# crockwell/rel_pose

Hardware: AMD Instinct MI355X
Metric: image-pairs/sec fwd+bwd @384x384, 1/2/4/8 MI355X; R,t err vs ref (higher is better)
Workload: dtype f32; 1 GPU; train.py step (ViTEss fwd + geodesic loss + bwd + grad all-reduce + clip + Adam), synthetic 384x384 pairs; scope=full, pairs_per_gpu=64, global_batch_pairs=64, parallelism=dp1, finite=True, gemm_operand_precision=exact fp32 MFMA, launch=eager

## Files before the change

__graft_entry__.py:

```python
import os
import subprocess
import sys

ROOT = os.path.dirname(os.path.abspath(__file__))
if ROOT not in sys.path:
    sys.path.insert(0, ROOT)


def build():
    import torch
    from rel_pose_amd import _build
    force = os.environ.get("RP_FORCE_BUILD", "" if torch.cuda.is_available() else "1") == "1"
    _build.build(force=force, verbose=True)
    from rel_pose_amd import _lib
    lib = _lib.load()
    assert lib.rp_abi_version() == _lib.ABI_VERSION and lib.rp_target_arch() == b"gfx950"
    assert lib.rp_abi_export_count() == _lib.ABI_EXPORTS == len(_lib.EXPORTS)
    assert _lib.load_readout().rp_readout_abi_version() == _lib.READOUT_ABI_VERSION
    assert _lib.load_eightpoint().rp_eightpoint_abi_version() == _lib.EIGHTPOINT_ABI_VERSION
    assert _lib.load_refine().rp_refine_abi_version() == _lib.REFINE_ABI_VERSION
    assert _lib.load_consensus().rp_consensus_abi_version() == _lib.CONSENSUS_ABI_VERSION
    assert _lib.load_submatch().rp_submatch_abi_version() == _lib.SUBMATCH_ABI_VERSION
    assert _lib.load_fivepoint().rp_fivepoint_abi_version() == _lib.FIVEPOINT_ABI_VERSION
    assert _lib.load_homography().rp_homography_abi_version() == _lib.HOMOGRAPHY_ABI_VERSION
    assert _lib.load_triangulate().rp_triangulate_abi_version() == _lib.TRIANGULATE_ABI_VERSION
    import rel_pose_amd.model
    import oracle.relpose_oracle
    print("build ok:", _lib.lib_path(), _build.READOUT_LIB, _build.EIGHTPOINT_LIB, _build.REFINE_LIB, _build.CONSENSUS_LIB, _build.SUBMATCH_LIB,
          _build.FIVEPOINT_LIB, _build.HOMOGRAPHY_LIB, _build.TRIANGULATE_LIB)


def smoke():
    import types

    import torch

    from oracle import relpose_oracle as O
    from rel_pose_amd import _lib
    from rel_pose_amd.model import ViTEss
    assert torch.cuda.is_available(), "smoke() needs cuda:0"
    _lib.load()
    torch.cuda.set_device(0)
    args = types.SimpleNamespace(noess="", pool_size=60, fc_hidden_size=512, fusion_transformer=True,
                                 transformer_depth=6, cross_features=False, use_single_softmax=False,
                                 no_pos_encoding=False, l1_pos_encoding=False)
    shapes = dict(O.vit_param_shapes())
    shapes.update(O.cnn_param_shapes())
    sd32, sd64 = O.make_state(shapes, torch.float32), O.make_state(shapes, torch.float64)
    model = ViTEss(args)
    model.load_state_dict(sd32)
    model = model.cuda().train()
    tok = O.synthetic_tokens(2)
    Gs = torch.tensor([0, 0, 0, 0, 0, 0, 1.0]).repeat(1, 2, 1)
    intr = torch.tensor([[30.0, 26.0, 12.0, 11.0]]).repeat(1, 2, 1)
    fmap = tok.permute(0, 2, 1).contiguous().view(2, 192, 24, 24).cuda().requires_grad_(True)
    out = model.forward_tokens(fmap, Gs.cuda(), intr.cuda())
    out[:, 1].square().sum().backward()
    t64 = tok.double().requires_grad_(True)
    ref = O.vit_ess_from_tokens(sd64, t64, Gs.double(), intr.double())
    ref[:, 1].square().sum().backward()
    t_err, q_err, ang = O.pose_errors(out.detach().cpu(), ref.detach())
    g_err = O.rel_err(fmap.grad.view(2, 192, 576).permute(0, 2, 1).cpu(), t64.grad)
# ... 10 lines not shown
```

rel_pose_amd/_build.py:

```python
import os
import subprocess
import sys

HERE = os.path.dirname(os.path.abspath(__file__))
CSRC = os.path.join(HERE, "csrc")
LIB = os.path.join(HERE, "librelpose_hip.so")
SOURCES = ["gemm.hip", "gemm_dma.hip", "rowwise.hip", "attention.hip", "attention_bf16.hip", "dw192_bf16.hip", "dw192_f32.hip", "dw192_split3.hip", "dx_lnbwd_bf16.hip", "emm.hip", "emm_bf16.hip", "batchnorm.hip", "se3loss.hip", "geom.hip", "augment.hip", "mlp_fused.hip", "linear_rows.hip", "conv_stem.hip", "conv_stem_bf16.hip", "conv_stem_wgrad_bf16.hip", "conv_stem_wgrad_f32.hip", "conv3x3_bf16.hip", "conv3x3_wgrad_bf16.hip", "conv3x3_wgrad_f32.hip", "conv3x3_f32.hip", "conv3x3_c128_f32.hip"]
READOUT_CSRC = os.path.join(HERE, "csrc_readout")
READOUT_LIB = os.path.join(HERE, "librelpose_readout.so")
READOUT_SOURCES = ["emm_readout.hip"]
EIGHTPOINT_CSRC = os.path.join(HERE, "csrc_eightpoint")
EIGHTPOINT_LIB = os.path.join(HERE, "librelpose_eightpoint.so")
EIGHTPOINT_SOURCES = ["eight_point.hip"]
REFINE_CSRC = os.path.join(HERE, "csrc_refine")
REFINE_LIB = os.path.join(HERE, "librelpose_refine.so")
REFINE_SOURCES = ["refine_pose.hip"]
CONSENSUS_CSRC = os.path.join(HERE, "csrc_consensus")
CONSENSUS_LIB = os.path.join(HERE, "librelpose_consensus.so")
CONSENSUS_SOURCES = ["consensus.hip"]
SUBMATCH_CSRC = os.path.join(HERE, "csrc_submatch")
SUBMATCH_LIB = os.path.join(HERE, "librelpose_submatch.so")
SUBMATCH_SOURCES = ["submatch.hip"]
FIVEPOINT_CSRC = os.path.join(HERE, "csrc_fivepoint")
FIVEPOINT_LIB = os.path.join(HERE, "librelpose_fivepoint.so")
FIVEPOINT_SOURCES = ["five_point.hip"]
HOMOGRAPHY_CSRC = os.path.join(HERE, "csrc_homography")
HOMOGRAPHY_LIB = os.path.join(HERE, "librelpose_homography.so")
HOMOGRAPHY_SOURCES = ["homography.hip"]
TRIANGULATE_CSRC = os.path.join(HERE, "csrc_triangulate")
TRIANGULATE_LIB = os.path.join(HERE, "librelpose_triangulate.so")
TRIANGULATE_SOURCES = ["triangulate.hip"]
ARCH = "gfx950"


def _hipcc():
    for c in (os.environ.get("HIPCC"), "/opt/rocm/bin/hipcc"):
        if c and os.path.exists(c):
            return c
    return "hipcc"


def _stale(lib, csrc, sources, headers):
    if not os.path.exists(lib):
        return True
    t = os.path.getmtime(lib)
    return any(os.path.getmtime(d) > t for d in [os.path.join(csrc, s) for s in sources] + headers)


def needs_build():
    return _stale(LIB, CSRC, SOURCES, _headers())


def readout_needs_build():
    return _stale(READOUT_LIB, READOUT_CSRC, READOUT_SOURCES, _readout_headers())


def eightpoint_needs_build():
    return _stale(EIGHTPOINT_LIB, EIGHTPOINT_CSRC, EIGHTPOINT_SOURCES, _eightpoint_headers())


def refine_needs_build():
    return _stale(REFINE_LIB, REFINE_CSRC, REFINE_SOURCES, _refine_headers())


def consensus_needs_build():
    return _stale(CONSENSUS_LIB, CONSENSUS_CSRC, CONSENSUS_SOURCES, _consensus_headers())


def submatch_needs_build():
    return _stale(SUBMATCH_LIB, SUBMATCH_CSRC, SUBMATCH_SOURCES, _submatch_headers())


def fivepoint_needs_build():
    return _stale(FIVEPOINT_LIB, FIVEPOINT_CSRC, FIVEPOINT_SOURCES, _fivepoint_headers())


def homography_needs_build():
    return _stale(HOMOGRAPHY_LIB, HOMOGRAPHY_CSRC, HOMOGRAPHY_SOURCES, _homography_headers())


def triangulate_needs_build():
    return _stale(TRIANGULATE_LIB, TRIANGULATE_CSRC, TRIANGULATE_SOURCES, _triangulate_headers())


def build(force=False, verbose=True):
    import fcntl
    with open(os.path.join(HERE, ".build.lock"), "w") as lock:
        fcntl.flock(lock, fcntl.LOCK_EX)
        try:
            if force or needs_build():
                _build_locked(verbose, force, LIB, CSRC, SOURCES, _headers())
            if force or readout_needs_build():
                _build_locked(verbose, force, READOUT_LIB, READOUT_CSRC, READOUT_SOURCES, _readout_headers())
            if force or eightpoint_needs_build():
                _build_locked(verbose, force, EIGHTPOINT_LIB, EIGHTPOINT_CSRC, EIGHTPOINT_SOURCES, _eightpoint_headers())
            if force or refine_needs_build():
                _build_locked(verbose, force, REFINE_LIB, REFINE_CSRC, REFINE_SOURCES, _refine_headers())
            if force or consensus_needs_build():
                _build_locked(verbose, force, CONSENSUS_LIB, CONSENSUS_CSRC, CONSENSUS_SOURCES, _consensus_headers())
            if force or submatch_needs_build():
                _build_locked(verbose, force, SUBMATCH_LIB, SUBMATCH_CSRC, SUBMATCH_SOURCES, _submatch_headers())
            if force or fivepoint_needs_build():
                _build_locked(verbose, force, FIVEPOINT_LIB, FIVEPOINT_CSRC, FIVEPOINT_SOURCES, _fivepoint_headers())
            if force or homography_needs_build():
                _build_locked(verbose, force, HOMOGRAPHY_LIB, HOMOGRAPHY_CSRC, HOMOGRAPHY_SOURCES, _homography_headers())
            if force or triangulate_needs_build():
                _build_locked(verbose, force, TRIANGULATE_LIB, TRIANGULATE_CSRC, TRIANGULATE_SOURCES, _triangulate_headers())
            return LIB
        finally:
            fcntl.flock(lock, fcntl.LOCK_UN)


def _headers():
    return [os.path.join(CSRC, h) for h in sorted(os.listdir(CSRC)) if h.endswith(".h")] + \
           [os.path.join(os.path.dirname(HERE), "include", "relpose_hip.h")]


def _readout_headers():
    return _headers() + [os.path.join(os.path.dirname(HERE), "include", "relpose_readout.h")]


def _eightpoint_headers():
    return _headers() + [os.path.join(os.path.dirname(HERE), "include", "relpose_eightpoint.h")]


def _refine_headers():
    return _headers() + [os.path.join(os.path.dirname(HERE), "include", "relpose_refine.h")]


def _consensus_headers():
    return _headers() + [os.path.join(os.path.dirname(HERE), "include", "relpose_consensus.h")]


def _submatch_headers():
    return _headers() + [os.path.join(os.path.dirname(HERE), "include", "relpose_submatch.h")]


def _fivepoint_headers():
    return _headers() + [os.path.join(os.path.dirname(HERE), "include", "relpose_fivepoint.h")]


def _homography_headers():
    return _headers() + [os.path.join(os.path.dirname(HERE), "include", "relpose_homography.h")]


def _triangulate_headers():
    return _headers() + [os.path.join(os.path.dirname(HERE), "include", "relpose_triangulate.h")]


def _build_locked(verbose, force, lib, csrc, sources, headers):
    cc = _hipcc()
    objs = []
    procs = []
    hdr_t = max(os.path.getmtime(h) for h in headers)
    for s in sources:
        o = os.path.join(csrc, s.replace(".hip", ".o"))
        objs.append(o)
        if not force and os.path.exists(o) and os.path.getmtime(o) > max(hdr_t, os.path.getmtime(os.path.join(csrc, s))):
            continue
        cmd = [cc, "--offload-arch=" + ARCH, "-O3", "-std=c++17", "-fPIC", "-c", os.path.join(csrc, s), "-o", o]
        if verbose:
            print(" ".join(cmd), flush=True)
        procs.append((s, subprocess.Popen(cmd, stdout=subprocess.PIPE, stderr=subprocess.STDOUT)))
    for s, p in procs:
        out, _ = p.communicate()
        if p.returncode != 0:
            sys.stderr.write(out.decode())
            raise RuntimeError("hipcc failed on " + s)
    tmp = lib + ".tmp.%d" % os.getpid()
    cmd = [cc, "--offload-arch=" + ARCH, "-shared", "-fPIC", "-o", tmp] + objs
    if verbose:
        print(" ".join(cmd), flush=True)
    subprocess.check_call(cmd)
    os.replace(tmp, lib)
    return lib


if __name__ == "__main__":
    build(force="--force" in sys.argv)
```

rel_pose_amd/_lib.py:

```python
import ctypes
import keyword
import os
import re
from ctypes import POINTER, Structure, c_char_p, c_float, c_int, c_longlong, c_size_t, c_void_p

import torch

from . import _build

_LIB = None
HEADER = os.path.join(os.path.dirname(os.path.dirname(os.path.abspath(__file__))), "include", "relpose_hip.h")

_SCALARS = {"int": c_int, "float": c_float, "long long": c_longlong, "size_t": c_size_t}
_POINTEES = ("void", "float", "double", "int", "unsigned char")
_DEFINE = re.compile(r"#\s*define\s+(RP_\w+)\s+(-?\d+|\(-?\d+\))")
_DECL = re.compile(r"(const\s+)?(unsigned\s+char|long\s+long|\w+)\s*(\*?)\s*([A-Za-z_]\w*(?:\s*,\s*[A-Za-z_]\w*)*)?")
_ITEM = re.compile(r"\s*(?:typedef\s+struct\s+(\w+)\s*\{([^{}]*);\s*\}\s*(\w+)\s*;"
                   r"|([\w\s*]+?)\b(rp_\w+)\s*\(([^()]*)\)\s*;"
                   r'|extern\s+"C"\s*\{|\})')


def _declaration(text, structs, header="relpose_hip.h"):
    m = _DECL.fullmatch(text.strip())
    if not m:
# ... 104 lines not shown
with open(SUBMATCH_HEADER) as _f:
    _SUBMATCH_CONSTS, _, _SUBMATCH_PROTOTYPES, _SUBMATCH_STATUS = _header_contract(_f.read(), "relpose_submatch.h")
SUBMATCH_ABI_VERSION = _SUBMATCH_CONSTS["RP_SUBMATCH_ABI_VERSION"]
SUBMATCH_EXPORTS = tuple(_SUBMATCH_PROTOTYPES)


_FIVEPOINT_LIB = None
FIVEPOINT_HEADER = os.path.join(os.path.dirname(HEADER), "relpose_fivepoint.h")
with open(FIVEPOINT_HEADER) as _f:
    _FIVEPOINT_CONSTS, _, _FIVEPOINT_PROTOTYPES, _FIVEPOINT_STATUS = _header_contract(_f.read(), "relpose_fivepoint.h")
FIVEPOINT_ABI_VERSION = _FIVEPOINT_CONSTS["RP_FIVEPOINT_ABI_VERSION"]
FIVEPOINT_MAX_P, FIVEPOINT_MAX_M, FIVEPOINT_ROOTS = (_FIVEPOINT_CONSTS[k] for k in ("RP_FIVEPOINT_MAX_P", "RP_FIVEPOINT_MAX_M", "RP_FIVEPOINT_ROOTS"))
FIVEPOINT_EXPORTS = tuple(_FIVEPOINT_PROTOTYPES)


_HOMOGRAPHY_LIB = None
HOMOGRAPHY_HEADER = os.path.join(os.path.dirname(HEADER), "relpose_homography.h")
with open(HOMOGRAPHY_HEADER) as _f:
    _HOMOGRAPHY_CONSTS, _, _HOMOGRAPHY_PROTOTYPES, _HOMOGRAPHY_STATUS = _header_contract(_f.read(), "relpose_homography.h")
HOMOGRAPHY_ABI_VERSION = _HOMOGRAPHY_CONSTS["RP_HOMOGRAPHY_ABI_VERSION"]
HOMOGRAPHY_MAX_P, HOMOGRAPHY_MAX_M, HOMOGRAPHY_MAX_ITERS = (_HOMOGRAPHY_CONSTS[k] for k in ("RP_HOMOGRAPHY_MAX_P", "RP_HOMOGRAPHY_MAX_M", "RP_HOMOGRAPHY_MAX_ITERS"))
HOMOGRAPHY_EXPORTS = tuple(_HOMOGRAPHY_PROTOTYPES)


_TRIANGULATE_LIB = None
TRIANGULATE_HEADER = os.path.join(os.path.dirname(HEADER), "relpose_triangulate.h")
with open(TRIANGULATE_HEADER) as _f:
    _TRIANGULATE_CONSTS, _, _TRIANGULATE_PROTOTYPES, _TRIANGULATE_STATUS = _header_contract(_f.read(), "relpose_triangulate.h")
TRIANGULATE_ABI_VERSION = _TRIANGULATE_CONSTS["RP_TRIANGULATE_ABI_VERSION"]
TRIANGULATE_MAX_P = _TRIANGULATE_CONSTS["RP_TRIANGULATE_MAX_P"]
TRIANGULATE_EXPORTS = tuple(_TRIANGULATE_PROTOTYPES)


def lib_path():
    return _build.LIB


def load():
    global _LIB
    if _LIB is not None:
        return _LIB
    path = _build.LIB
    if _build.needs_build():
        _build.build(verbose=False)
    try:
        lib = ctypes.CDLL(path)
    except OSError as e:
        raise RuntimeError("rel_pose_amd: cannot load HIP extension %s (%s); there is no CPU fallback" % (path, e))
    lib.rp_abi_version.restype = c_int
    if lib.rp_abi_version() != ABI_VERSION:
        raise RuntimeError("rel_pose_amd: %s has ABI version %d, this package binds version %d -- rebuild with "
                           "`python -m rel_pose_amd._build --force`" % (path, lib.rp_abi_version(), ABI_VERSION))
    if len(EXPORTS) != ABI_EXPORTS:
        raise RuntimeError("rel_pose_amd: include/relpose_hip.h declares %d entry points (RP_ABI_EXPORTS = %d)" % (len(EXPORTS), ABI_EXPORTS))
    lib.rp_abi_export_count.restype = c_int
    if lib.rp_abi_export_count() != ABI_EXPORTS:
        raise RuntimeError("rel_pose_amd: %s was compiled with %d entry points, the header declares %d -- rebuild"
                           % (path, lib.rp_abi_export_count(), ABI_EXPORTS))
    for name, (res, args) in _PROTOTYPES.items():
        fn = getattr(lib, name)
        fn.restype = res
        fn.argtypes = args
        if name in _STATUS:
            fn.errcheck = _raise_on_status
    _LIB = lib
    return lib
# ... 169 lines not shown
        fn.restype = res
        fn.argtypes = args
        if name in _HOMOGRAPHY_STATUS:
            fn.errcheck = _raise_on_status
    _HOMOGRAPHY_LIB = lib
    return lib


def load_triangulate():
    global _TRIANGULATE_LIB
    if _TRIANGULATE_LIB is not None:
        return _TRIANGULATE_LIB
    path = _build.TRIANGULATE_LIB
    if _build.triangulate_needs_build():
        _build.build(verbose=False)
    try:
        lib = ctypes.CDLL(path)
    except OSError as e:
        raise RuntimeError("rel_pose_amd: cannot load HIP extension %s (%s); there is no CPU fallback" % (path, e))
    lib.rp_triangulate_abi_version.restype = c_int
    if lib.rp_triangulate_abi_version() != TRIANGULATE_ABI_VERSION:
        raise RuntimeError("rel_pose_amd: %s has ABI version %d, this package binds version %d -- rebuild with "
                           "`python -m rel_pose_amd._build --force`" % (path, lib.rp_triangulate_abi_version(), TRIANGULATE_ABI_VERSION))
    for name, (res, args) in _TRIANGULATE_PROTOTYPES.items():
        fn = getattr(lib, name)
        fn.restype = res
        fn.argtypes = args
        if name in _TRIANGULATE_STATUS:
            fn.errcheck = _raise_on_status
    _TRIANGULATE_LIB = lib
    return lib


def _raise_on_status(rc, func, args):
    check(rc, func.__name__)
    return rc


def check(rc, what):
    if rc != 0:
        if rc < 0:
            raise RuntimeError("rel_pose_amd: %s failed: %s (RP error %d)" % (what, RP_ERRORS.get(rc, "?"), rc))
        raise RuntimeError("rel_pose_amd: %s failed: hipError %d" % (what, rc))
```

rel_pose_amd/csrc/dw192_f32.hip:

```cpp
#include "common.h"
#include "../../include/relpose_hip.h"

namespace {

constexpr int W = 192;
constexpr int SR = 32;
constexpr int ST_FL = SR * W;

struct DwF {
  const float* a; const float* b; float* ws;
  int M, N, lda, rows_per_split, nsplit;
};

__global__ __launch_bounds__(256, 1) void dw192_f32_kernel(DwF p) {
  __shared__ __attribute__((aligned(16))) float As[2][ST_FL];
  __shared__ __attribute__((aligned(16))) float Bs[2][ST_FL];
  const int tid = threadIdx.x, lane = tid & 63, wave = __builtin_amdgcn_readfirstlane(tid >> 6), l31 = lane & 31, hi = lane >> 5;
  const int ntile = p.N / W;
  const int nt = (blockIdx.x >> 3) % ntile, sp = ((blockIdx.x >> 3) / ntile) * 8 + (blockIdx.x & 7);
  if (sp >= p.nsplit) return;
  const int m0 = sp * p.rows_per_split;
  const int m1 = min(p.M, m0 + p.rows_per_split);
  const int nst = (m1 - m0) / SR;
  const float* ab = p.a + (long long)m0 * p.lda + nt * W;
  const float* bb = p.b + (long long)m0 * W;

  unsigned aoff[6], boff[6];
#pragma unroll
  for (int i = 0; i < 6; ++i) {
    const int byte = (wave + 4 * i) * 1024 + lane * 16;
    const int r = byte / 768, c = byte % 768;
    aoff[i] = (unsigned)(r * p.lda * 4 + c);
    boff[i] = (unsigned)(r * W * 4 + c);
  }
  const unsigned as0 = lds_byte_addr(&As[0][0]) + wave * 1024, bs0 = lds_byte_addr(&Bs[0][0]) + wave * 1024;
  auto issue = [&](int s, int buf) {
    const void* sa = uniform_ptr(ab + (long long)s * SR * p.lda);
    const void* sb = uniform_ptr(bb + (long long)s * SR * W);
#pragma unroll
    for (int i = 0; i < 6; ++i) glds16(sa, aoff[i], as0 + buf * (ST_FL * 4) + i * 4096);
#pragma unroll
    for (int i = 0; i < 6; ++i) glds16(sb, boff[i], bs0 + buf * (ST_FL * 4) + i * 4096);
  };

  const int wr = wave >> 1, wc = wave & 1;
  const int ao = hi * W + 96 * wr + l31, bo = hi * W + 96 * wc + l31;
  f32x16 acc[3][3];
#pragma unroll
  for (int i = 0; i < 3; ++i)
#pragma unroll
    for (int j = 0; j < 3; ++j) acc[i][j] = zero16();

  if (nst > 0) issue(0, 0);
  asm volatile("s_waitcnt vmcnt(0)" ::: "memory");
  __builtin_amdgcn_s_barrier();
  for (int s = 0; s < nst; ++s) {
    const int buf = s & 1;
    const int sn = min(s + 1, nst - 1);
    const void* sa = uniform_ptr(ab + (long long)sn * SR * p.lda);
    const void* sb = uniform_ptr(bb + (long long)sn * SR * W);
    const unsigned an0 = as0 + (buf ^ 1) * (ST_FL * 4), bn0 = bs0 + (buf ^ 1) * (ST_FL * 4);
    const unsigned at = lds_byte_addr(As[buf] + ao), bt = lds_byte_addr(Bs[buf] + bo);
    float af[3], bf[3];
    static_for<3>([&](auto i) {
      af[i] = lds_rd32<128 * i>(at);
      bf[i] = lds_rd32<128 * i>(bt);
    });
    static_for<SR / 2>([&](auto tt) {
      constexpr int t = tt;
      asm volatile("s_waitcnt lgkmcnt(0)" : "+v"(af[0]), "+v"(af[1]), "+v"(af[2]), "+v"(bf[0]), "+v"(bf[1]), "+v"(bf[2]));
      float an[3], bn[3];
      if constexpr (t + 1 < SR / 2) {
        static_for<3>([&](auto i) {
          an[i] = lds_rd32<(2 * (t + 1) * W + 32 * i) * 4>(at);
          bn[i] = lds_rd32<(2 * (t + 1) * W + 32 * i) * 4>(bt);
        });
      }
      if (t < 6) glds16(sa, aoff[t < 6 ? t : 0], an0 + t * 4096);
      else if (t < 12) glds16(sb, boff[t >= 6 && t < 12 ? t - 6 : 0], bn0 + (t - 6) * 4096);
      __builtin_amdgcn_sched_barrier(0);
#pragma unroll
      for (int i = 0; i < 3; ++i)
#pragma unroll
        for (int j = 0; j < 3; ++j) acc[i][j] = mfma32(af[i], bf[j], acc[i][j]);
      if constexpr (t + 1 < SR / 2) {
#pragma unroll
        for (int i = 0; i < 3; ++i) {
          af[i] = an[i];
          bf[i] = bn[i];
        }
      }
    });
    asm volatile("s_waitcnt vmcnt(0) lgkmcnt(0)" ::: "memory");
    __builtin_amdgcn_s_barrier();
  }
  float* slab = p.ws + (long long)sp * p.N * W + (long long)(nt * W + 96 * wr) * W + 96 * wc + l31;
#pragma unroll
  for (int i = 0; i < 3; ++i)
#pragma unroll
    for (int j = 0; j < 3; ++j)
#pragma unroll
      for (int r = 0; r < 16; ++r) slab[(long long)(32 * i + acc_row(r, hi)) * W + 32 * j] = acc[i][j][r];
}

}

extern "C" int rp_dw192_f32_splits(int M, int N) {
  if (M <= 0 || N <= 0 || N % W) return 0;
  const int ntile = N / W, stages = M / SR;
  int sp = 8 * (32 / ntile);
  if (sp > stages) sp = stages;
  if (sp < 2) sp = 2;
  const int per = (stages + sp - 1) / sp;
  sp = (stages + per - 1) / per;
  return sp < 2 ? 2 : sp;
}

extern "C" size_t rp_dw192_f32_workspace_bytes(int M, int N) {
  return (size_t)rp_dw192_f32_splits(M, N) * (size_t)N * W * sizeof(float);
}

extern "C" int rp_dw192_f32(const float* a, int lda, const float* b, int M, int N, void* workspace, size_t workspace_bytes, void* stream) {
  if (!a || !b || !workspace || M <= 0 || N <= 0) return RP_EBADSHAPE;
  if (N % W || M % SR || M < 2 * SR || (lda & 3) || lda < N) return RP_EBADSHAPE;
  if (((uintptr_t)a | (uintptr_t)b | (uintptr_t)workspace) & 15) return RP_EALIGN;
  if (workspace_bytes < rp_dw192_f32_workspace_bytes(M, N)) return RP_EWORKSPACE;
  DwF p;
  p.a = a; p.b = b; p.ws = (float*)workspace; p.M = M; p.N = N; p.lda = lda;
  p.nsplit = rp_dw192_f32_splits(M, N);
  const int stages = M / SR;
  p.rows_per_split = ((stages + p.nsplit - 1) / p.nsplit) * SR;
  const dim3 grid((N / W) * ((p.nsplit + 7) / 8) * 8);
  hipLaunchKernelGGL(dw192_f32_kernel, grid, dim3(256), 0, (hipStream_t)stream, p);
  RP_CHECK_LAUNCH();
  return RP_OK;
// ... 2 lines not shown
```

rel_pose_amd/ops.py:

```python
import ctypes
import itertools
import math
import os
import threading

import torch

from . import _lib

N_TOK = 576
DIM = 192
HEADS = 3
LN_EPS = 1e-6
XW = 96
GW = 224
NWG = 6


def _chk(*ts):
    for t in ts:
        if t is None:
            continue
        if not (t.is_cuda and t.dtype == torch.float32 and t.is_contiguous()):
            raise RuntimeError("rel_pose_amd ops need contiguous fp32 GPU tensors (no CPU fallback exists); got "
# ... 551 lines not shown
        np_ = 3 if add is not None else 2
        part = _empty(-(-M // lib.rp_dx_lnbwd_bf16_tile_rows()), np_ * DIM, like=x)
        dx = torch.empty_like(x)
        wt = bf16_weight(transposed(W))
        with timed("dx_lnbwd_bf16", 2.0 * M * N * DIM, M * (2.0 * N + 4.0 * DIM * (3 if add is not None else 2))):
            lib.rp_dx_lnbwd_bf16(_p(dy), _p(wt), _p(x), _p(gamma), _p(mean), _p(rstd), _p(add), _p(dx), _p(part), M, N, _st())
        sums = colsum(part)
        if add is None:
            return dx, sums[:DIM], sums[DIM:]
        return dx, sums[:DIM], sums[DIM:2 * DIM], sums[2 * DIM:]
    np_ = 3 if add is not None else 2
    part = _empty(-(-M // 64), np_ * DIM, like=dy)
    dx = gemm(dy, W, M, DIM, N, b_layout=1, residual=add, ln=(x, mean, rstd, gamma, part))
    sums = colsum(part)
    if add is None:
        return dx, sums[:DIM], sums[DIM:]
    return dx, sums[:DIM], sums[DIM:2 * DIM], sums[2 * DIM:]


DW192 = os.environ.get("RP_DW192", "1") == "1"


DW192_F32 = os.environ.get("RP_DW192_F32", "1") == "1"
DW_SPLIT3 = os.environ.get("RP_DW_SPLIT3", "0") == "1"


def _dw192(a, b, out, trans):
    lib = _lib.load()
    M, N = a.shape
    f32 = a.dtype == torch.float32
    sk = (lib.rp_dw192_f32_splits if f32 else lib.rp_dw192_bf16_splits)(M, N)
    nbytes = (lib.rp_dw192_f32_workspace_bytes if f32 else lib.rp_dw192_bf16_workspace_bytes)(M, N)
    deferred = (_sk_batch() is not None and torch.cuda.current_stream(a.device).cuda_stream == _sk_batch()[2])
    ws = _arena_take(nbytes, a.device, _sk_batch()[1]) if deferred else _workspace(nbytes, a.device)
    if f32 and DW_SPLIT3:
        with timed("dw192_split3", 2.0 * M * N * DIM, 4.0 * (M * (N + DIM) + sk * N * DIM)):
            lib.rp_dw192_split3(_p(a), N, _p(b), M, N, _p(ws), nbytes, _st())
    elif f32:
        with timed("dw192_f32", 2.0 * M * N * DIM, 4.0 * (M * (N + DIM) + sk * N * DIM)):
            lib.rp_dw192_f32(_p(a), N, _p(b), M, N, _p(ws), nbytes, _st())
    else:
        with timed("dw192_bf16" if b.dtype == torch.bfloat16 else "dw192_bf16_f32b", 2.0 * M * N * DIM,
                   M * (2.0 * N + b.element_size() * DIM) + 4.0 * sk * N * DIM):
            lib.rp_dw192_bf16(_p(a), N, _p(b), 1 if b.dtype == torch.float32 else 0, M, N, _p(ws), nbytes, _st())
    task = (ws, out, N, DIM, N if trans else DIM, sk, trans)
    if deferred:
        _sk_batch()[0].append(task)
    else:
        arr = (_lib.RpSplitkTask * 1)()
        arr[0].ws, arr[0].C, arr[0].M, arr[0].N, arr[0].ldc, arr[0].split_k, arr[0].trans_c = ws.data_ptr(), out.data_ptr(), N, DIM, task[4], sk, 1 if trans else 0
        lib.rp_splitk_reduce_multi(arr, 1, _st())
    return out


def linear_dw(dy, x):
    M, N = dy.shape
    K = x.shape[1]
    if DW192 and GEMM_PRECISION == 1 and M % 64 == 0 and M >= 4096 and dy.is_contiguous() and x.is_contiguous():
        bfd = torch.bfloat16
        if dy.dtype == bfd and N % DIM == 0 and K == DIM and (N >= K or x.dtype != bfd):
            return _dw192(dy, x, torch.empty(N, K, device=dy.device, dtype=torch.float32), False)
        if x.dtype == bfd and K % DIM == 0 and N == DIM:
            return _dw192(x, dy, torch.empty(N, K, device=dy.device, dtype=torch.float32), True)
    if (DW192_F32 and GEMM_PRECISION == 0 and M % 32 == 0 and M >= 4096 and dy.dtype == torch.float32 and x.dtype == torch.float32
            and dy.is_contiguous() and x.is_contiguous()):
        if N % DIM == 0 and K == DIM and N >= K:
            return _dw192(dy, x, torch.empty(N, K, device=dy.device, dtype=torch.float32), False)
        if K % DIM == 0 and N == DIM:
            return _dw192(x, dy, torch.empty(N, K, device=dy.device, dtype=torch.float32), True)
    if x.dtype != torch.float32 and not (K > N and M >= 4096):
        x = x.float()
    if dy.dtype != torch.float32 and K > N and M >= 4096:
        dy = dy.float()
    if K > N and M >= 4096:
        sk = max(2, pick_split_k(K, N, M, 1, 1))
        out = _empty(N, K, like=dy)
        return gemm(x, dy, K, N, M, a_layout=1, b_layout=1, out=out, ldc=K, split_k=sk, trans_c=True, defer=True)
    return gemm(dy, x, N, K, M, a_layout=1, b_layout=1, defer=True)


COLSUM_BATCHING = True
_COLSUM_BATCH = None
_COLSUM_STREAM = None


# ... 658 lines not shown
        x = x.contiguous()
        Z = x.shape[0]
        x2 = x.view(Z * N_TOK, DIM)
        bfp = _bf16_path()
        pst = mrun = None
        if bfp:
            qkv, xn1, m1, r1 = ln_linear(x2, n1w, n1b, qkv_w, qkv_b, train=train, out_dtype=torch.bfloat16, xn_dtype=torch.bfloat16)
            o, lse = attn_fwd_bf16(qkv, Z, k_xor=3 if cross else 0)
        else:
            qkv, xn1, m1, r1 = ln_linear(x2, n1w, n1b, qkv_w, qkv_b, train=train)
            if train and ATTN_STORE_P and ATTN_BWD_STORE_DS and not cross and not ATTN_BF16 and not USE_SIDE_STREAM:
                o, lse, pst, mrun = attn_fwd(qkv, Z, save_p=True)
            else:
                o, lse = attn_fwd(qkv, Z, k_xor=3 if cross else 0)
        ctx.cross = cross
        x1 = linear(o, proj_w, proj_b, residual=x2)
        y, xn2, m2, r2, h, hpre = _mlp_block_fwd(x1, n2w, n2b, fc1_w, fc1_b, fc2_w, fc2_b, train)
        if train:
            register_transposed(proj_w, fc1_w, fc2_w)
            if bfp:
                register_transposed(qkv_w)
            ctx.save_for_backward(x2, m1, r1, xn1, qkv, o, lse, x1, m2, r2, xn2, h, hpre, n1w, qkv_w, proj_w, n2w,
                                  fc1_w, fc2_w, pst, mrun)
            ctx.Z = Z
        return y.view(Z, N_TOK, DIM)

    @staticmethod
    def backward(ctx, dy):
        (x2, m1, r1, xn1, qkv, o, lse, x1, m2, r2, xn2, h, hpre, n1w, qkv_w, proj_w, n2w, fc1_w,
         fc2_w, pst, mrun) = ctx.saved_tensors
        Z = ctx.Z
        dy = dy.contiguous().view(Z * N_TOK, DIM)
        fork = _Fork(dy.device)
        with colsum_batch(), splitk_batch():
            (dx1, dn2w, dn2b, dfc2b), dfc1w, dfc1b, dfc2w, _ = _mlp_bwd(fork, dy, xn2, h, hpre, fc1_w, fc2_w, want_db2=False,
                                                                         ln=(x1, n2w, m2, r2, dy))
            fork.sync_side()
            dprojw = fork.on_side(lambda: linear_dw(dx1, o))
            if qkv.dtype == torch.bfloat16:
                do = linear_dx(dx1, proj_w, out_dtype=torch.bfloat16)
                dqkv, bpart = attn_bwd_bf16(qkv, o, lse, do, Z, kv_xor=1 if ctx.cross else 0, want_bias_partials=True)
            else:
                do = linear_dx(dx1, proj_w)
                dqkv, bpart = attn_bwd(qkv, o, lse, do, Z, fork, kv_xor=1 if ctx.cross else 0, want_bias_partials=True,
                                       saved_p=None if pst is None else (pst, mrun))
            fork.sync_main()
            fork.sync_side()
            if bpart is not None:
                dqkvw, dqkvb = fork.on_side(lambda: linear_dw(dqkv, xn1)), colsum(bpart)
            else:
                dqkvw, dqkvb = _param_grads(fork, dqkv, xn1)
            dx, dn1w, dn1b, dprojb = linear_dx_lnbwd(dqkv, qkv_w, x2, n1w, m1, r1, add=dx1)
            fork.sync_main()
        return (dx.view(Z, N_TOK, DIM), dn1w, dn1b, dqkvw, dqkvb, dprojw, dprojb, dn2w, dn2b, dfc1w, dfc1b, dfc2w,
                dfc2b, None)


class CrossBlockFn(_Fn):

    @staticmethod
    def forward(ctx, x, pos, n1w, n1b, qkv_w, qkv_b, pf_w, pf_b, n2w, n2b, fc1_w, fc1_b, fc2_w, fc2_b, single=False,
                cross=False):
        train = _train(ctx)
        x = x.contiguous()
        Z = x.shape[0]
        x2 = x.view(Z * N_TOK, DIM)
        ctx.single, ctx.cross = single, cross
        sc = None
        if _bf16_path() and not single and not cross:
            qkv, xn, m1, r1 = ln_linear(x2, n1w, n1b, qkv_w, qkv_b, train=train, out_dtype=torch.bfloat16, xn_dtype=torch.bfloat16)
            g, (xa, t, rlse, clse) = emm_forward_bf16(qkv, pos, Z)
        else:
            qkv, xn, m1, r1 = ln_linear(x2, n1w, n1b, qkv_w, qkv_b, train=train)
            rlse, clse, sc = emm_stats(qkv, Z, single, want_s=True)
            xa = emm_build_x(qkv, pos, Z)
            t, fpart = emm_apply(qkv, xa, rlse, clse, Z, swap=False, want_t=train, single=single,
                                 x_left=xa if cross else None, s=sc)
            g = emm_finalize(fpart, Z)
        pf_wp = _padded(pf_w, (0, GW - pf_w.shape[1]))
        f = linear(g, pf_wp, pf_b)
        y, fn, m2, r2, h, hpre = _mlp_block_fwd(f, n2w, n2b, fc1_w, fc1_b, fc2_w, fc2_b, train)
        if train:
            register_transposed(fc1_w, fc2_w)
            if qkv.dtype == torch.bfloat16:
                register_transposed(qkv_w)
            ctx.save_for_backward(x2, m1, r1, xn, qkv, rlse, clse, xa, t, g, f, m2, r2, fn, h, hpre, n1w, qkv_w, pf_wp,
                                  n2w, fc1_w, fc2_w, sc)
            ctx.Z = Z
            ctx.pf_cols = pf_w.shape[1]
        return y.view(Z, 70, DIM)

    @staticmethod
    def backward(ctx, dy):
        (x2, m1, r1, xn, qkv, rlse, clse, xa, t, g, f, m2, r2, fn, h, hpre, n1w, qkv_w, pf_wp, n2w, fc1_w,
         fc2_w, sc) = ctx.saved_tensors
        Z = ctx.Z
        dy = dy.contiguous().view(Z * 70, DIM)
        fork = _Fork(dy.device)
        with colsum_batch(), splitk_batch():
            (df_, dn2w, dn2b, dfc2b), dfc1w, dfc1b, dfc2w, _ = _mlp_bwd(fork, dy, fn, h, hpre, fc1_w, fc2_w, want_db2=False,
                                                                         ln=(f, n2w, m2, r2, dy))
            fork.sync_side()
            dpfw_full, dpfb = _param_grads(fork, df_, g)
            dg = linear_dx(df_, pf_wp)
            dF = emm_finalize_bwd(dg, Z)
            if qkv.dtype == torch.bfloat16:
                dqkv = emm_backward_bf16(qkv, xa, t, rlse, clse, dF, Z)
                fork.sync_side()
                dqkvw = fork.on_side(lambda: linear_dw(dqkv, xn))
                dqkvb = dqkv.sum(0, dtype=torch.float32)
            else:
                dqkv = emm_backward(qkv, xa, t, rlse, clse, dF, Z, single=ctx.single, cross=ctx.cross, s=sc)
                fork.sync_side()
                dqkvw, dqkvb = _param_grads(fork, dqkv, xn)
            dx, dn1w, dn1b = linear_dx_lnbwd(dqkv, qkv_w, x2, n1w, m1, r1)
            fork.sync_main()
        dpfw = dpfw_full[:, :ctx.pf_cols].contiguous()
        return (dx.view(Z, N_TOK, DIM), None, dn1w, dn1b, dqkvw, dqkvb, dpfw, dpfb, dn2w, dn2b, dfc1w, dfc1b, dfc2w,
                dfc2b, None, None)


def _regress_fwd(feats, gs, w0, b0, w2, b2, w4, b4):
    lib = _lib.load()
    B = feats.shape[0]
    h1 = linear(feats, w0, b0, act=2)
    h2 = linear(h1, w2, b2, act=2)
    w4p = _padded(w4, (0, 0, 0, 2))
    b4p = _padded(b4, (0, 2))
    pred = linear(h2, w4p, b4p)[:, :14].contiguous()
    gs = gs.contiguous()
    _chk(gs)
    out = _empty(B, 2, 7, like=feats)
# ... 847 lines not shown
```

Baseline: 1990 image-pairs/sec.

## Batch deferred f32 weight-gradient GEMMs into one grouped XCD-aware launch

Deferred fp32 dW kernels (192-wide weight gradients) inside transformer-block backward passes are now queued rather than launched one by one. On exit they go out as a single grouped kernel whose host-side planner picks split-K per problem to fill 256 workgroups and places tiles across the 8 XCDs. This cuts launch count and raises occupancy for small individual dW GEMMs. The costs are a deferred dependency on side-stream ordering and some host planning overhead per batch.

```diff
diff --git a/__graft_entry__.py b/__graft_entry__.py
--- a/__graft_entry__.py
+++ b/__graft_entry__.py
@@ -24,10 +24,11 @@
     assert _lib.load_fivepoint().rp_fivepoint_abi_version() == _lib.FIVEPOINT_ABI_VERSION
     assert _lib.load_homography().rp_homography_abi_version() == _lib.HOMOGRAPHY_ABI_VERSION
     assert _lib.load_triangulate().rp_triangulate_abi_version() == _lib.TRIANGULATE_ABI_VERSION
+    assert _lib.load_dwbatch().rp_dwbatch_abi_version() == _lib.DWBATCH_ABI_VERSION
     import rel_pose_amd.model
     import oracle.relpose_oracle
     print("build ok:", _lib.lib_path(), _build.READOUT_LIB, _build.EIGHTPOINT_LIB, _build.REFINE_LIB, _build.CONSENSUS_LIB, _build.SUBMATCH_LIB,
-          _build.FIVEPOINT_LIB, _build.HOMOGRAPHY_LIB, _build.TRIANGULATE_LIB)
+          _build.FIVEPOINT_LIB, _build.HOMOGRAPHY_LIB, _build.TRIANGULATE_LIB, _build.DWBATCH_LIB)
 
 
 def smoke():
diff --git a/include/relpose_dwbatch.h b/include/relpose_dwbatch.h
--- /dev/null
+++ b/include/relpose_dwbatch.h
@@ -0,0 +1,30 @@
+#ifndef RELPOSE_DWBATCH_H
+#define RELPOSE_DWBATCH_H
+
+#include "relpose_hip.h"
+
+#ifdef __cplusplus
+extern "C" {
+#endif
+
+#define RP_DWBATCH_ABI_VERSION 1
+#define RP_DWBATCH_MAX 8
+#define RP_DWBATCH_WORKGROUPS 256
+int rp_dwbatch_abi_version(void);
+
+typedef struct RpDwProblem {
+  const float* a;
+  const float* b;
+  float* ws;
+  size_t ws_bytes;
+  int M, N, lda, split;
+} RpDwProblem;
+
+int rp_dw192_f32_batch_plan(RpDwProblem* problems, int n);
+
+int rp_dw192_f32_batch(const RpDwProblem* problems, int n, void* stream);
+
+#ifdef __cplusplus
+}
+#endif
+#endif
diff --git a/rel_pose_amd/_build.py b/rel_pose_amd/_build.py
--- a/rel_pose_amd/_build.py
+++ b/rel_pose_amd/_build.py
@@ -30,6 +30,9 @@
 TRIANGULATE_CSRC = os.path.join(HERE, "csrc_triangulate")
 TRIANGULATE_LIB = os.path.join(HERE, "librelpose_triangulate.so")
 TRIANGULATE_SOURCES = ["triangulate.hip"]
+DWBATCH_CSRC = os.path.join(HERE, "csrc_dwbatch")
+DWBATCH_LIB = os.path.join(HERE, "librelpose_dwbatch.so")
+DWBATCH_SOURCES = ["dw192_f32_batch.hip"]
 ARCH = "gfx950"
 
 
@@ -83,6 +86,10 @@
     return _stale(TRIANGULATE_LIB, TRIANGULATE_CSRC, TRIANGULATE_SOURCES, _triangulate_headers())
 
 
+def dwbatch_needs_build():
+    return _stale(DWBATCH_LIB, DWBATCH_CSRC, DWBATCH_SOURCES, _dwbatch_headers())
+
+
 def build(force=False, verbose=True):
     import fcntl
     with open(os.path.join(HERE, ".build.lock"), "w") as lock:
@@ -106,6 +113,8 @@
                 _build_locked(verbose, force, HOMOGRAPHY_LIB, HOMOGRAPHY_CSRC, HOMOGRAPHY_SOURCES, _homography_headers())
             if force or triangulate_needs_build():
                 _build_locked(verbose, force, TRIANGULATE_LIB, TRIANGULATE_CSRC, TRIANGULATE_SOURCES, _triangulate_headers())
+            if force or dwbatch_needs_build():
+                _build_locked(verbose, force, DWBATCH_LIB, DWBATCH_CSRC, DWBATCH_SOURCES, _dwbatch_headers())
             return LIB
         finally:
             fcntl.flock(lock, fcntl.LOCK_UN)
@@ -148,6 +157,10 @@
     return _headers() + [os.path.join(os.path.dirname(HERE), "include", "relpose_triangulate.h")]
 
 
+def _dwbatch_headers():
+    return _headers() + [os.path.join(os.path.dirname(HERE), "include", "relpose_dwbatch.h")]
+
+
 def _build_locked(verbose, force, lib, csrc, sources, headers):
     cc = _hipcc()
     objs = []
diff --git a/rel_pose_amd/_lib.py b/rel_pose_amd/_lib.py
--- a/rel_pose_amd/_lib.py
+++ b/rel_pose_amd/_lib.py
@@ -160,6 +160,16 @@
 TRIANGULATE_EXPORTS = tuple(_TRIANGULATE_PROTOTYPES)
 
 
+_DWBATCH_LIB = None
+DWBATCH_HEADER = os.path.join(os.path.dirname(HEADER), "relpose_dwbatch.h")
+with open(DWBATCH_HEADER) as _f:
+    _DWBATCH_CONSTS, _DWBATCH_STRUCTS, _DWBATCH_PROTOTYPES, _DWBATCH_STATUS = _header_contract(_f.read(), "relpose_dwbatch.h")
+DWBATCH_ABI_VERSION = _DWBATCH_CONSTS["RP_DWBATCH_ABI_VERSION"]
+DWBATCH_MAX, DWBATCH_WORKGROUPS = _DWBATCH_CONSTS["RP_DWBATCH_MAX"], _DWBATCH_CONSTS["RP_DWBATCH_WORKGROUPS"]
+RpDwProblem = _DWBATCH_STRUCTS["RpDwProblem"]
+DWBATCH_EXPORTS = tuple(_DWBATCH_PROTOTYPES)
+
+
 def lib_path():
     return _build.LIB
 
@@ -395,6 +405,31 @@
     return lib
 
 
+def load_dwbatch():
+    global _DWBATCH_LIB
+    if _DWBATCH_LIB is not None:
+        return _DWBATCH_LIB
+    path = _build.DWBATCH_LIB
+    if _build.dwbatch_needs_build():
+        _build.build(verbose=False)
+    try:
+        lib = ctypes.CDLL(path)
+    except OSError as e:
+        raise RuntimeError("rel_pose_amd: cannot load HIP extension %s (%s); there is no CPU fallback" % (path, e))
+    lib.rp_dwbatch_abi_version.restype = c_int
+    if lib.rp_dwbatch_abi_version() != DWBATCH_ABI_VERSION:
+        raise RuntimeError("rel_pose_amd: %s has ABI version %d, this package binds version %d -- rebuild with "
+                           "`python -m rel_pose_amd._build --force`" % (path, lib.rp_dwbatch_abi_version(), DWBATCH_ABI_VERSION))
+    for name, (res, args) in _DWBATCH_PROTOTYPES.items():
+        fn = getattr(lib, name)
+        fn.restype = res
+        fn.argtypes = args
+        if name in _DWBATCH_STATUS:
+            fn.errcheck = _raise_on_status
+    _DWBATCH_LIB = lib
+    return lib
+
+
 def _raise_on_status(rc, func, args):
     check(rc, func.__name__)
     return rc
diff --git a/rel_pose_amd/csrc/dw192_f32.hip b/rel_pose_amd/csrc/dw192_f32.hip
--- a/rel_pose_amd/csrc/dw192_f32.hip
+++ b/rel_pose_amd/csrc/dw192_f32.hip
@@ -1,11 +1,10 @@
-#include "common.h"
+#include "dw192_f32_stream.h"
 #include "../../include/relpose_hip.h"
 
 namespace {
 
-constexpr int W = 192;
-constexpr int SR = 32;
-constexpr int ST_FL = SR * W;
+using dw192f32::SR;
+using dw192f32::W;
 
 struct DwF {
   const float* a; const float* b; float* ws;
@@ -13,94 +12,14 @@
 };
 
 __global__ __launch_bounds__(256, 1) void dw192_f32_kernel(DwF p) {
-  __shared__ __attribute__((aligned(16))) float As[2][ST_FL];
-  __shared__ __attribute__((aligned(16))) float Bs[2][ST_FL];
-  const int tid = threadIdx.x, lane = tid & 63, wave = __builtin_amdgcn_readfirstlane(tid >> 6), l31 = lane & 31, hi = lane >> 5;
   const int ntile = p.N / W;
   const int nt = (blockIdx.x >> 3) % ntile, sp = ((blockIdx.x >> 3) / ntile) * 8 + (blockIdx.x & 7);
   if (sp >= p.nsplit) return;
   const int m0 = sp * p.rows_per_split;
   const int m1 = min(p.M, m0 + p.rows_per_split);
   const int nst = (m1 - m0) / SR;
-  const float* ab = p.a + (long long)m0 * p.lda + nt * W;
-  const float* bb = p.b + (long long)m0 * W;
-
-  unsigned aoff[6], boff[6];
-#pragma unroll
-  for (int i = 0; i < 6; ++i) {
-    const int byte = (wave + 4 * i) * 1024 + lane * 16;
-    const int r = byte / 768, c = byte % 768;
-    aoff[i] = (unsigned)(r * p.lda * 4 + c);
-    boff[i] = (unsigned)(r * W * 4 + c);
-  }
-  const unsigned as0 = lds_byte_addr(&As[0][0]) + wave * 1024, bs0 = lds_byte_addr(&Bs[0][0]) + wave * 1024;
-  auto issue = [&](int s, int buf) {
-    const void* sa = uniform_ptr(ab + (long long)s * SR * p.lda);
-    const void* sb = uniform_ptr(bb + (long long)s * SR * W);
-#pragma unroll
-    for (int i = 0; i < 6; ++i) glds16(sa, aoff[i], as0 + buf * (ST_FL * 4) + i * 4096);
-#pragma unroll
-    for (int i = 0; i < 6; ++i) glds16(sb, boff[i], bs0 + buf * (ST_FL * 4) + i * 4096);
-  };
-
-  const int wr = wave >> 1, wc = wave & 1;
-  const int ao = hi * W + 96 * wr + l31, bo = hi * W + 96 * wc + l31;
-  f32x16 acc[3][3];
-#pragma unroll
-  for (int i = 0; i < 3; ++i)
-#pragma unroll
-    for (int j = 0; j < 3; ++j) acc[i][j] = zero16();
-
-  if (nst > 0) issue(0, 0);
-  asm volatile("s_waitcnt vmcnt(0)" ::: "memory");
-  __builtin_amdgcn_s_barrier();
-  for (int s = 0; s < nst; ++s) {
-    const int buf = s & 1;
-    const int sn = min(s + 1, nst - 1);
-    const void* sa = uniform_ptr(ab + (long long)sn * SR * p.lda);
-    const void* sb = uniform_ptr(bb + (long long)sn * SR * W);
-    const unsigned an0 = as0 + (buf ^ 1) * (ST_FL * 4), bn0 = bs0 + (buf ^ 1) * (ST_FL * 4);
-    const unsigned at = lds_byte_addr(As[buf] + ao), bt = lds_byte_addr(Bs[buf] + bo);
-    float af[3], bf[3];
-    static_for<3>([&](auto i) {
-      af[i] = lds_rd32<128 * i>(at);
-      bf[i] = lds_rd32<128 * i>(bt);
-    });
-    static_for<SR / 2>([&](auto tt) {
-      constexpr int t = tt;
-      asm volatile("s_waitcnt lgkmcnt(0)" : "+v"(af[0]), "+v"(af[1]), "+v"(af[2]), "+v"(bf[0]), "+v"(bf[1]), "+v"(bf[2]));
-      float an[3], bn[3];
-      if constexpr (t + 1 < SR / 2) {
-        static_for<3>([&](auto i) {
-          an[i] = lds_rd32<(2 * (t + 1) * W + 32 * i) * 4>(at);
-          bn[i] = lds_rd32<(2 * (t + 1) * W + 32 * i) * 4>(bt);
-        });
-      }
-      if (t < 6) glds16(sa, aoff[t < 6 ? t : 0], an0 + t * 4096);
-      else if (t < 12) glds16(sb, boff[t >= 6 && t < 12 ? t - 6 : 0], bn0 + (t - 6) * 4096);
-      __builtin_amdgcn_sched_barrier(0);
-#pragma unroll
-      for (int i = 0; i < 3; ++i)
-#pragma unroll
-        for (int j = 0; j < 3; ++j) acc[i][j] = mfma32(af[i], bf[j], acc[i][j]);
-      if constexpr (t + 1 < SR / 2) {
-#pragma unroll
-        for (int i = 0; i < 3; ++i) {
-          af[i] = an[i];
-          bf[i] = bn[i];
-        }
-      }
-    });
-    asm volatile("s_waitcnt vmcnt(0) lgkmcnt(0)" ::: "memory");
-    __builtin_amdgcn_s_barrier();
-  }
-  float* slab = p.ws + (long long)sp * p.N * W + (long long)(nt * W + 96 * wr) * W + 96 * wc + l31;
-#pragma unroll
-  for (int i = 0; i < 3; ++i)
-#pragma unroll
-    for (int j = 0; j < 3; ++j)
-#pragma unroll
-      for (int r = 0; r < 16; ++r) slab[(long long)(32 * i + acc_row(r, hi)) * W + 32 * j] = acc[i][j][r];
+  dw192f32::stream_tile(p.a + (long long)m0 * p.lda + nt * W, p.lda, p.b + (long long)m0 * W, nst,
+                        p.ws + (long long)sp * p.N * W + (long long)(nt * W) * W);
 }
 
 }
diff --git a/rel_pose_amd/csrc/dw192_f32_stream.h b/rel_pose_amd/csrc/dw192_f32_stream.h
--- /dev/null
+++ b/rel_pose_amd/csrc/dw192_f32_stream.h
@@ -0,0 +1,93 @@
+#pragma once
+#include "common.h"
+
+namespace dw192f32 {
+
+constexpr int W = 192;
+constexpr int SR = 32;
+constexpr int ST_FL = SR * W;
+
+RP_DEV void stream_tile(const float* ab, int lda, const float* bb, int nst, float* tile) {
+  __shared__ __attribute__((aligned(16))) float As[2][ST_FL];
+  __shared__ __attribute__((aligned(16))) float Bs[2][ST_FL];
+  const int tid = threadIdx.x, lane = tid & 63, wave = __builtin_amdgcn_readfirstlane(tid >> 6), l31 = lane & 31, hi = lane >> 5;
+
+  unsigned aoff[6], boff[6];
+#pragma unroll
+  for (int i = 0; i < 6; ++i) {
+    const int byte = (wave + 4 * i) * 1024 + lane * 16;
+    const int r = byte / 768, c = byte % 768;
+    aoff[i] = (unsigned)(r * lda * 4 + c);
+    boff[i] = (unsigned)(r * W * 4 + c);
+  }
+  const unsigned as0 = lds_byte_addr(&As[0][0]) + wave * 1024, bs0 = lds_byte_addr(&Bs[0][0]) + wave * 1024;
+  auto issue = [&](int s, int buf) {
+    const void* sa = uniform_ptr(ab + (long long)s * SR * lda);
+    const void* sb = uniform_ptr(bb + (long long)s * SR * W);
+#pragma unroll
+    for (int i = 0; i < 6; ++i) glds16(sa, aoff[i], as0 + buf * (ST_FL * 4) + i * 4096);
+#pragma unroll
+    for (int i = 0; i < 6; ++i) glds16(sb, boff[i], bs0 + buf * (ST_FL * 4) + i * 4096);
+  };
+
+  const int wr = wave >> 1, wc = wave & 1;
+  const int ao = hi * W + 96 * wr + l31, bo = hi * W + 96 * wc + l31;
+  f32x16 acc[3][3];
+#pragma unroll
+  for (int i = 0; i < 3; ++i)
+#pragma unroll
+    for (int j = 0; j < 3; ++j) acc[i][j] = zero16();
+
+  if (nst > 0) issue(0, 0);
+  asm volatile("s_waitcnt vmcnt(0)" ::: "memory");
+  __builtin_amdgcn_s_barrier();
+  for (int s = 0; s < nst; ++s) {
+    const int buf = s & 1;
+    const int sn = min(s + 1, nst - 1);
+    const void* sa = uniform_ptr(ab + (long long)sn * SR * lda);
+    const void* sb = uniform_ptr(bb + (long long)sn * SR * W);
+    const unsigned an0 = as0 + (buf ^ 1) * (ST_FL * 4), bn0 = bs0 + (buf ^ 1) * (ST_FL * 4);
+    const unsigned at = lds_byte_addr(As[buf] + ao), bt = lds_byte_addr(Bs[buf] + bo);
+    float af[3], bf[3];
+    static_for<3>([&](auto i) {
+      af[i] = lds_rd32<128 * i>(at);
+      bf[i] = lds_rd32<128 * i>(bt);
+    });
+    static_for<SR / 2>([&](auto tt) {
+      constexpr int t = tt;
+      asm volatile("s_waitcnt lgkmcnt(0)" : "+v"(af[0]), "+v"(af[1]), "+v"(af[2]), "+v"(bf[0]), "+v"(bf[1]), "+v"(bf[2]));
+      float an[3], bn[3];
+      if constexpr (t + 1 < SR / 2) {
+        static_for<3>([&](auto i) {
+          an[i] = lds_rd32<(2 * (t + 1) * W + 32 * i) * 4>(at);
+          bn[i] = lds_rd32<(2 * (t + 1) * W + 32 * i) * 4>(bt);
+        });
+      }
+      if (t < 6) glds16(sa, aoff[t < 6 ? t : 0], an0 + t * 4096);
+      else if (t < 12) glds16(sb, boff[t >= 6 && t < 12 ? t - 6 : 0], bn0 + (t - 6) * 4096);
+      __builtin_amdgcn_sched_barrier(0);
+#pragma unroll
+      for (int i = 0; i < 3; ++i)
+#pragma unroll
+        for (int j = 0; j < 3; ++j) acc[i][j] = mfma32(af[i], bf[j], acc[i][j]);
+      if constexpr (t + 1 < SR / 2) {
+#pragma unroll
+        for (int i = 0; i < 3; ++i) {
+          af[i] = an[i];
+          bf[i] = bn[i];
+        }
+      }
+    });
+    asm volatile("s_waitcnt vmcnt(0) lgkmcnt(0)" ::: "memory");
+    __builtin_amdgcn_s_barrier();
+  }
+  float* out = tile + (long long)(96 * wr) * W + 96 * wc + l31;
+#pragma unroll
+  for (int i = 0; i < 3; ++i)
+#pragma unroll
+    for (int j = 0; j < 3; ++j)
+#pragma unroll
+      for (int r = 0; r < 16; ++r) out[(long long)(32 * i + acc_row(r, hi)) * W + 32 * j] = acc[i][j][r];
+}
+
+}
diff --git a/rel_pose_amd/csrc_dwbatch/dw192_f32_batch.hip b/rel_pose_amd/csrc_dwbatch/dw192_f32_batch.hip
--- /dev/null
+++ b/rel_pose_amd/csrc_dwbatch/dw192_f32_batch.hip
@@ -0,0 +1,150 @@
+#include "../csrc/dw192_f32_stream.h"
+#include "../../include/relpose_dwbatch.h"
+
+namespace {
+
+using dw192f32::SR;
+using dw192f32::W;
+
+constexpr int WGS = RP_DWBATCH_WORKGROUPS, XCDS = 8, PER_XCD = WGS / XCDS;
+constexpr unsigned IDLE = 0xffffffffu;
+
+struct DwB {
+  struct {
+    const float* a; const float* b; float* ws;
+    int M, N, lda, rows_per_split;
+  } pr[RP_DWBATCH_MAX];
+  unsigned table[WGS];
+};
+
+__global__ __launch_bounds__(256, 1) void dw192_f32_kernel(DwB p) {
+  const unsigned e = p.table[blockIdx.x];
+  if (e == IDLE) return;
+  const int q = e & 15, nt = (e >> 4) & 255, sp = e >> 12;
+  const float* a = p.pr[q].a;
+  const float* b = p.pr[q].b;
+  float* ws = p.pr[q].ws;
+  const int M = p.pr[q].M, N = p.pr[q].N, lda = p.pr[q].lda, rps = p.pr[q].rows_per_split;
+  const int m0 = sp * rps;
+  const int m1 = min(M, m0 + rps);
+  const int nst = (m1 - m0) / SR;
+  dw192f32::stream_tile(a + (long long)m0 * lda + nt * W, lda, b + (long long)m0 * W, nst,
+                        ws + (long long)sp * N * W + (long long)(nt * W) * W);
+}
+
+int tight(int stages, int sp) {
+  const int per = (stages + sp - 1) / sp;
+  return (stages + per - 1) / per;
+}
+
+int plan(const int* M, const int* N, int n, int* split) {
+  if (n < 1 || n > RP_DWBATCH_MAX) return 0;
+  long long T = 0;
+  int tiles_all = 0;
+  for (int p = 0; p < n; ++p) {
+    if (M[p] < 2 * SR || M[p] % SR || N[p] < W || N[p] % W) return 0;
+    T += (long long)(N[p] / W) * (M[p] / SR);
+    tiles_all += N[p] / W;
+  }
+  if (2 * tiles_all > WGS) return 0;
+  auto total = [&] {
+    int s = 0;
+    for (int p = 0; p < n; ++p) s += (N[p] / W) * split[p];
+    return s;
+  };
+  for (int p = 0; p < n; ++p) {
+    const int stages = M[p] / SR;
+    long long sp = (long long)stages * WGS / T;
+    if (sp > stages) sp = stages;
+    if (sp < 2) sp = 2;
+    split[p] = tight(stages, (int)sp);
+  }
+  while (total() > WGS) {
+    int best = 0;
+    for (int p = 0; p < n; ++p) {
+      const int per = (M[p] / SR + split[p] - 1) / split[p];
+      if (split[p] > 2 && (best == 0 || per < best)) best = per;
+    }
+    if (best == 0) return 0;
+    for (int p = 0; p < n; ++p) {
+      const int stages = M[p] / SR;
+      if (split[p] > 2 && (stages + split[p] - 1) / split[p] == best) split[p] = tight(stages, split[p] - 1);
+    }
+  }
+  return total();
+}
+
+int place(const int* N, const int* split, int n, unsigned* table) {
+  int used[XCDS] = {};
+  for (int b = 0; b < WGS; ++b) table[b] = IDLE;
+  int widest = 0;
+  for (int p = 0; p < n; ++p) widest = N[p] / W > widest ? N[p] / W : widest;
+  for (int w = widest; w >= 1; --w)
+    for (int p = 0; p < n; ++p) {
+      if (N[p] / W != w) continue;
+      for (int sp = 0; sp < split[p]; ++sp) {
+        int x = 0;
+        for (int y = 1; y < XCDS; ++y)
+          if (used[y] < used[x]) x = y;
+        const bool whole = used[x] + w <= PER_XCD;
+        for (int nt = 0; nt < w; ++nt) {
+          if (!whole) {
+            x = 0;
+            for (int y = 1; y < XCDS; ++y)
+              if (used[y] < used[x]) x = y;
+          }
+          table[used[x]++ * XCDS + x] = (unsigned)p | (unsigned)nt << 4 | (unsigned)sp << 12;
+        }
+      }
+    }
+  int slots = 0;
+  for (int x = 0; x < XCDS; ++x) slots = used[x] > slots ? used[x] : slots;
+  return slots * XCDS;
+}
+
+}
+
+extern "C" int rp_dwbatch_abi_version(void) { return RP_DWBATCH_ABI_VERSION; }
+
+extern "C" int rp_dw192_f32_batch_plan(RpDwProblem* problems, int n) {
+  if (!problems || n < 1 || n > RP_DWBATCH_MAX) return 0;
+  int M[RP_DWBATCH_MAX], N[RP_DWBATCH_MAX], split[RP_DWBATCH_MAX];
+  for (int p = 0; p < n; ++p) {
+    M[p] = problems[p].M;
+    N[p] = problems[p].N;
+  }
+  const int wgs = plan(M, N, n, split);
+  if (wgs)
+    for (int p = 0; p < n; ++p) problems[p].split = split[p];
+  return wgs;
+}
+
+extern "C" int rp_dw192_f32_batch(const RpDwProblem* problems, int n, void* stream) {
+  if (!problems || n < 1 || n > RP_DWBATCH_MAX) return RP_EBADSHAPE;
+  int M[RP_DWBATCH_MAX], N[RP_DWBATCH_MAX], split[RP_DWBATCH_MAX];
+  for (int p = 0; p < n; ++p) {
+    const RpDwProblem& d = problems[p];
+    if (!d.a || !d.b || !d.ws || d.M <= 0 || d.N <= 0 || (d.lda & 3) || d.lda < d.N) return RP_EBADSHAPE;
+    M[p] = d.M;
+    N[p] = d.N;
+  }
+  if (!plan(M, N, n, split)) return RP_EBADSHAPE;
+  for (int p = 0; p < n; ++p)
+    if (problems[p].split != split[p]) return RP_EBADSHAPE;
+  for (int p = 0; p < n; ++p)
+    if (((uintptr_t)problems[p].a | (uintptr_t)problems[p].b | (uintptr_t)problems[p].ws) & 15) return RP_EALIGN;
+  for (int p = 0; p < n; ++p)
+    if (problems[p].ws_bytes < (size_t)split[p] * (size_t)N[p] * W * sizeof(float)) return RP_EWORKSPACE;
+  DwB k;
+  for (int p = 0; p < RP_DWBATCH_MAX; ++p) {
+    const RpDwProblem& d = problems[p < n ? p : 0];
+    const int stages = d.M / SR, sp = split[p < n ? p : 0];
+    k.pr[p].a = d.a; k.pr[p].b = d.b; k.pr[p].ws = d.ws;
+    k.pr[p].M = d.M; k.pr[p].N = d.N; k.pr[p].lda = d.lda;
+    k.pr[p].rows_per_split = ((stages + sp - 1) / sp) * SR;
+  }
+  const int grid = place(N, split, n, k.table);
+  hipLaunchKernelGGL(dw192_f32_kernel, dim3(grid), dim3(256), 0, (hipStream_t)stream, k);
+  RP_CHECK_LAUNCH();
+  return RP_OK;
+}
diff --git a/rel_pose_amd/ops.py b/rel_pose_amd/ops.py
--- a/rel_pose_amd/ops.py
+++ b/rel_pose_amd/ops.py
@@ -607,6 +607,10 @@
     sk = (lib.rp_dw192_f32_splits if f32 else lib.rp_dw192_bf16_splits)(M, N)
     nbytes = (lib.rp_dw192_f32_workspace_bytes if f32 else lib.rp_dw192_bf16_workspace_bytes)(M, N)
     deferred = (_sk_batch() is not None and torch.cuda.current_stream(a.device).cuda_stream == _sk_batch()[2])
+    dwb = getattr(_TLS, "dw_batch", None)
+    if f32 and not DW_SPLIT3 and deferred and dwb is not None and dwb[1] is _sk_batch():
+        dwb[0].append((a, b, out, trans))
+        return out
     ws = _arena_take(nbytes, a.device, _sk_batch()[1]) if deferred else _workspace(nbytes, a.device)
     if f32 and DW_SPLIT3:
         with timed("dw192_split3", 2.0 * M * N * DIM, 4.0 * (M * (N + DIM) + sk * N * DIM)):
@@ -626,6 +630,44 @@
         arr[0].ws, arr[0].C, arr[0].M, arr[0].N, arr[0].ldc, arr[0].split_k, arr[0].trans_c = ws.data_ptr(), out.data_ptr(), N, DIM, task[4], sk, 1 if trans else 0
         lib.rp_splitk_reduce_multi(arr, 1, _st())
     return out
+
+
+DW_BATCH = os.environ.get("RP_DW_BATCH", "1") == "1"
+
+
+class dw_batch:
+
+    def __enter__(self):
+        self.prev = getattr(_TLS, "dw_batch", None)
+        sk = _sk_batch()
+        _TLS.dw_batch = ([], sk) if (DW_BATCH and sk is not None) else None
+        return self
+
+    def __exit__(self, et, ev, tb):
+        cur, _TLS.dw_batch = _TLS.dw_batch, self.prev
+        if et is None and cur and cur[0]:
+            for i in range(0, len(cur[0]), _lib.DWBATCH_MAX):
+                _dw192_f32_batch(cur[0][i:i + _lib.DWBATCH_MAX], cur[1])
+        return False
+
+
+def _dw192_f32_batch(items, sk_batch):
+    lib = _lib.load_dwbatch()
+    arr = (_lib.RpDwProblem * len(items))()
+    for p, (a, b, _, _) in zip(arr, items):
+        p.a, p.b, p.M, p.N, p.lda = a.data_ptr(), b.data_ptr(), a.shape[0], a.shape[1], a.shape[1]
+    if not lib.rp_dw192_f32_batch_plan(arr, len(items)):
+        raise RuntimeError("rel_pose_amd: rp_dw192_f32_batch_plan refused the shapes %s" % [tuple(a.shape) for a, _, _, _ in items])
+    flops = nbytes = 0.0
+    for p, (a, b, out, trans) in zip(arr, items):
+        p.ws_bytes = 4 * p.split * p.N * DIM
+        ws = _arena_take(p.ws_bytes, a.device, sk_batch[1])
+        p.ws = ws.data_ptr()
+        flops += 2.0 * p.M * p.N * DIM
+        nbytes += 4.0 * (p.M * (p.N + DIM) + p.split * p.N * DIM)
+        sk_batch[0].append((ws, out, p.N, DIM, p.N if trans else DIM, p.split, trans))
+    with timed("dw192_f32", flops, nbytes):
+        lib.rp_dw192_f32_batch(arr, len(items), _st())
 
 
 def linear_dw(dy, x):
@@ -1350,7 +1392,7 @@
         Z = ctx.Z
         dy = dy.contiguous().view(Z * N_TOK, DIM)
         fork = _Fork(dy.device)
-        with colsum_batch(), splitk_batch():
+        with colsum_batch(), splitk_batch(), dw_batch():
             (dx1, dn2w, dn2b, dfc2b), dfc1w, dfc1b, dfc2w, _ = _mlp_bwd(fork, dy, xn2, h, hpre, fc1_w, fc2_w, want_db2=False,
                                                                          ln=(x1, n2w, m2, r2, dy))
             fork.sync_side()
@@ -1415,7 +1457,7 @@
         Z = ctx.Z
         dy = dy.contiguous().view(Z * 70, DIM)
         fork = _Fork(dy.device)
-        with colsum_batch(), splitk_batch():
+        with colsum_batch(), splitk_batch(), dw_batch():
             (df_, dn2w, dn2b, dfc2b), dfc1w, dfc1b, dfc2w, _ = _mlp_bwd(fork, dy, fn, h, hpre, fc1_w, fc2_w, want_db2=False,
                                                                          ln=(f, n2w, m2, r2, dy))
             fork.sync_side()
```

Measured after the change: 2004 image-pairs/sec, median of 6. No clear change (+0.7%).
